# wondras/ld-decode

Hardware: AMD Instinct MI355X
Metric: RF Msamples/s (40 MSPS NTSC, full RF->.tbc decode) (higher is better)
Workload: dtype f64

## Files before the change

include/ldgpu.h:

```cpp
#ifndef LDGPU_H
#define LDGPU_H

#include <stdint.h>
#include <stddef.h>

#ifdef __cplusplus
extern "C" {
#endif

#define LDG_OK 0
#define LDG_EINVAL (-1)
#define LDG_EDEVICE (-2)
#define LDG_ENOMEM (-3)
#define LDG_ESTATE (-4)

#define LDG_SYSTEM_NTSC 0
#define LDG_SYSTEM_PAL 1

#define LDG_FMT_U8 0
#define LDG_FMT_S16 1
#define LDG_FMT_R30 2
#define LDG_FMT_LDS 3

#define LDG_FS_VALID 0
// ... 74 lines not shown
int ldg_stream_release(ldg_ctx* ctx, int64_t below_sample);
int ldg_stream_seek(ldg_ctx* ctx, int64_t first_sample);
int ldg_stream_window(ldg_ctx* ctx, int64_t* out4);
int ldg_stream_stats(ldg_ctx* ctx, double* out, int n);
int ldg_stream_close(ldg_ctx* ctx);

int ldg_decode_reads(ldg_ctx* ctx, int n, const int64_t* read_starts, const double* mtf, const int32_t* slots,
                     ldg_field_info* info);
int ldg_decode_reads_async(ldg_ctx* ctx, int n, const int64_t* read_starts, const double* mtf,
                           const int32_t* slots);
#define LDG_READ_FULL 1
#define LDG_READ_PROBE 2
int ldg_decode_reads_async2(ldg_ctx* ctx, int n, const int64_t* read_starts, const double* mtf,
                            const int32_t* slots, uint8_t* full);
int ldg_set_video_cut(ldg_ctx* ctx, int64_t out_samples);
int ldg_decode_reads_wait(ldg_ctx* ctx, ldg_field_info* info);

int ldg_field_audio(ldg_ctx* ctx, int n, const int32_t* slots, const double* offsets, int16_t* pcm,
                    int64_t pcm_stride, int32_t* counts, double* next_offsets);

int ldg_field_audio_async(ldg_ctx* ctx, int n, const int32_t* slots, const double* offsets);
int ldg_field_audio_collect(ldg_ctx* ctx, int16_t* pcm, int64_t pcm_stride, int32_t* counts, double* next_offsets);

int ldg_archive_fields(ldg_ctx* ctx, int n, const int32_t* slots, int64_t first);
int ldg_archive_audio(ldg_ctx* ctx, int n, const int64_t* entries, const double* offsets, int16_t* pcm,
                      int64_t pcm_stride, int32_t* counts, double* next_offsets);
int ldg_audio_offsets(double o0, int64_t n, const double* linecounts, double line_period, double* out);

int ldg_assemble_frames(ldg_ctx* ctx, int n, const int32_t* top_slots, const int32_t* bottom_slots,
                        uint16_t* out, int out_is_device);
// ... 105 lines not shown
```

ld-decode_amd/csrc/abi.inc:

```
#include <hip/hip_runtime.h>
#include <algorithm>
#include <chrono>
#include <thread>
#include <cmath>
#include <complex>
#include <cstdio>
#include <cstring>
#include <map>
#include <string>
#include <vector>

namespace {

using namespace ldg;

struct DevBuf {
  void* p = nullptr;
  size_t n = 0;
};

}

static inline comb::CombOpt comb_defaults() {
  comb::CombOpt c;
// ... 834 lines not shown
  return check_launch(ctx, "ldg_k_demod");
}

static int launch_chain(ldg_ctx* ctx, hipStream_t st, int n, const int32_t* M_) {
  const SysConst C = ctx->C;
  if (!(ctx->skip >> 0 & 1)) LDG_LAUNCH_ON(st, "sync_walk", ldg_k_sync_walk, n * SEG_K, 64, M_, ctx->d_reads, ctx->video, ctx->vread, ctx->vchan, C,
             ctx->d_status, ctx->d_npos, ctx->d_npk, ctx->d_nlv, ctx->d_ncnt, ctx->d_stile, ctx->d_sst,
             ctx->d_sbits);
  if (!(ctx->skip >> 1 & 1)) LDG_LAUNCH_ON(st, "sync", ldg_k_sync, n, 64, M_, ctx->d_reads, ctx->video, ctx->vread, ctx->vchan, C, ctx->d_recs,
             ctx->d_peaks, ctx->d_status, ctx->d_npos, ctx->d_npk, ctx->d_nlv, ctx->d_ncnt, ctx->d_stile,
             ctx->d_sst, ctx->d_sbits, (ctx->skip >> 9) & 1);
  if (!(ctx->skip >> 2 & 1)) LDG_LAUNCH_ON(st, "linelocs", ldg_k_linelocs, n, 64, M_, ctx->video, ctx->vread, ctx->vchan, C, ctx->d_recs,
             ctx->d_peaks, ctx->d_lines, ctx->d_bad, ctx->d_sst, ctx->d_sbits);
  const dim3 g_lines((unsigned)(C.frame_lines / 2 + 5), (unsigned)n), g_rows((unsigned)(C.frame_lines / 2 + 1), (unsigned)n);
  if (!(ctx->skip >> 3 & 1)) LDG_LAUNCH_ON(st, "hsync_lines", ldg_k_hsync_lines, g_lines, 64, M_, ctx->video, ctx->vread, ctx->vchan, C,
             ctx->d_recs, ctx->d_lines, ctx->d_bad);
  if (!(ctx->skip >> 4 & 1)) LDG_LAUNCH_ON(st, "hsync_field", ldg_k_hsync_field, n, 256, M_, C, ctx->d_recs, ctx->d_lines, ctx->d_bad);
  if (!(ctx->skip >> 5 & 1)) LDG_LAUNCH_ON(st, "philips", ldg_k_philips, n, 192, M_, ctx->video, ctx->vread, ctx->vchan, C, ctx->d_recs,
             ctx->d_lines, ctx->d_reads);
  if (int rc = check_launch(ctx, "field kernels")) return rc;
  if (ctx->system == 0) {
    for (int pass = 0; pass < 2; pass++) {
      if (!(ctx->skip >> 6 & 1)) LDG_LAUNCH_ON(st, "burst_lines", ldg_k_burst_lines, g_lines, 64, M_, ctx->video, ctx->vread, ctx->vchan, C,
                 ctx->d_recs, ctx->d_lines, ctx->d_blevel, pass, ctx->d_bst, ctx->d_reads);
      if (!(ctx->skip >> 7 & 1)) LDG_LAUNCH_ON(st, "burst_field", ldg_k_burst_field, n, 64, M_, ctx->video, ctx->vread, ctx->vchan,
                 ctx->d_recs, ctx->d_lines, ctx->d_blevel, C, pass, ctx->d_bst);
    }
  } else {
    LDG_LAUNCH_ON(st, "pilot_lines", ldg_k_pilot_lines, g_lines, 64, M_, ctx->video, ctx->vread, ctx->vchan, C,
               ctx->d_recs, ctx->d_lines, ctx->d_scratch, ctx->d_reads);
    LDG_LAUNCH_ON(st, "pilot_field", ldg_k_pilot_field, n, 256, M_, ctx->d_recs, ctx->d_lines, C, ctx->d_scratch);
  }
  if (!(ctx->skip >> 8 & 1)) LDG_LAUNCH_ON(st, "final_lines", ldg_k_final_lines, g_rows, FINAL_NT, M_, ctx->video, ctx->vread, ctx->vchan, C,
             ctx->d_recs, ctx->d_lines, ctx->d_blevel, ctx->d_pic, ctx->pic_stride, ctx->d_reads);
  if (int rc = check_launch(ctx, "tbc kernels")) return rc;
  return LDG_OK;
}

struct HostProf {
  bool on = getenv("LDG_HOSTPROF") != nullptr;
  std::chrono::steady_clock::time_point t0 = std::chrono::steady_clock::now(), t = t0;
  char buf[512];
  int len = 0;
  void mark(const char* what) {
    if (!on) return;
    const auto u = std::chrono::steady_clock::now();
// ... 14 lines not shown

int ldg_set_video_cut(ldg_ctx* ctx, int64_t out_samples) {
  if (!ctx || out_samples < 0) return LDG_EINVAL;
  ctx->video_cut = out_samples;
  return LDG_OK;
}

static void read_geometry(ReadDesc& r, int64_t start) {
  r.readsample = start;
  r.end = start + READLEN + 1;
  r.s0 = start > BLOCKCUT ? start - BLOCKCUT : 0;
  r.n_out = (int32_t)(r.end - r.s0 + 1);
  r.n_blocks = (int32_t)((r.end - r.s0 + BLOCKSTEP - 1) / BLOCKSTEP);
  r.n_audio = (int32_t)((r.end - r.s0) / AUDIO_DIV1 + 1);
  r.n_audio2 = r.n_audio / AUDIO_DIV2;
}

static int probe_halfwin(const SysConst& C) { return (int)(3 * (int64_t)C.linelen / 10); }

int ldg_decode_reads_async2(ldg_ctx* ctx, int n, const int64_t* read_starts, const double* mtf,
                            const int32_t* slots, uint8_t* full) {
  if (!ctx || n <= 0 || n > ctx->max_reads || !read_starts || !mtf) return LDG_EINVAL;
  if (ctx->ncalls >= ldg_ctx::MAX_CALLS) {
    ctx->err = "too many decodes outstanding";
    return LDG_ESTATE;
  }
  if (!ctx->have_filters || !ctx->cap) {
    ctx->err = "filters or capture not set";
    return LDG_ESTATE;
  }
// ... 73 lines not shown
      if (!(full[i] & LDG_READ_PROBE)) continue;
      ReadDesc pr = nr[i];
      const int64_t r0 = nr[i].readsample - PROBE_C;
      if (!(ctx->stages & 1) || r0 - BLOCKCUT < ctx->cap_first ||
          r0 - BLOCKCUT + BLOCKLEN > ctx->cap_first + ctx->cap_nsamp) {
        full[i] &= (uint8_t)~LDG_READ_PROBE;
        continue;
      }
      read_geometry(pr, r0);
      pr.end = r0 + BLOCKSTEP + 64;
      pr.n_out = (int32_t)(pr.end - pr.s0 + 1);
      pr.n_blocks = 1;
      pr.n_audio = (int32_t)((pr.end - pr.s0) / AUDIO_DIV1 + 1);
      pr.n_audio2 = pr.n_audio / AUDIO_DIV2;
      pr.vcut = 0;
      hpr[np] = pr;
      hps[np++] = smap[i];
    }
  int32_t* dps = ctx->d_psm + (size_t)ci * R;
  hipStream_t sp = ctx->sprep;
  if (call.demod_recorded) LDG_TRY(hipStreamWaitEvent(sp, call.ev_demod, 0));
  LDG_LAUNCH_ON(sp, "new_reads", ldg_k_new_reads, (n + 255) / 256, 256, hnr, hsm, n, dsm, ctx->d_reads, ctx->d_status);
  if (np) LDG_LAUNCH_ON(sp, "new_reads", ldg_k_new_reads, (np + 255) / 256, 256, hpr, hps, np, dps, ctx->d_preads,
                        ctx->d_status);
    LDG_LAUNCH_ON(sp, "rf_table", ldg_k_rf_table, dim3(BLOCKLEN / 256, (unsigned)tm.size()), 256, ctx->rfvideo, ctx->mtf,
                  ctx->mtf_logabs, ctx->mtf_arg, htm, ctx->rf_cur);
  if (int rc = check_launch(ctx, "ldg_k_rf_table")) return rc;
  LDG_TRY(hipEventRecord(call.ev_prep, sp));
  LDG_TRY(hipStreamWaitEvent(s, call.ev_prep, 0));
  if (ctx->frames_recorded && ctx->frames_demod) LDG_TRY(hipStreamWaitEvent(s, ctx->ev_frames, 0));
// ... 1663 lines not shown
```

ld-decode_amd/csrc/common.hpp:

```cpp
#pragma once
#include <stdint.h>

namespace ldg {

constexpr int BLOCKLEN = 16384;
constexpr int BLOCKCUT = 1024;
constexpr int BLOCKCUT_END = 32;
constexpr int BLOCKSTEP = BLOCKLEN - BLOCKCUT - BLOCKCUT_END;
constexpr int HALF = BLOCKLEN / 2;
constexpr int MAX_BLOCKS_PER_READ = 66;
constexpr int PARK_SLOTS = 2048;
constexpr int PARK_EXTRA = 64;
constexpr int PARK_SCRATCH = PARK_SLOTS + PARK_EXTRA;
constexpr int PARK_TOTAL = PARK_SCRATCH + 1;
constexpr int PARK_OWNERS = PARK_SLOTS + PARK_EXTRA;
constexpr int READLEN = 1000000;
constexpr int MAX_NOUT = READLEN + 1026 + 16;
constexpr int AUDIO_DIV1 = 16;
constexpr int AUDIO_BLOCK = 1024;
constexpr int MAX_NAUDIO = MAX_NOUT / AUDIO_DIV1 + 16;
constexpr int AUDIO_DIV2 = 4;
constexpr int AUDIO2_BLOCK = 4096;
constexpr int MAX_NAUDIO2 = MAX_NAUDIO / AUDIO_DIV2 + 16;
constexpr int MAX_PEAKS = 2048;
// ... 16 lines not shown
  FS_CRASH = 6,
  FS_PENDING = 7,
  FS_MIGRATED = 8,
  FS_VCUT = 9,
};

struct ReadDesc {
  int64_t readsample;
  int64_t s0;
  int64_t end;
  int32_t n_out;
  int32_t n_blocks;
  int32_t n_audio;
  int32_t n_audio2;
  int32_t filt_slot;
  int32_t pad_;
  int64_t vcut;
};

struct SysConst {
  double freq_hz;
  double freq;
  double ire0, hz_ire, vsync_ire;
  double sync_lo, sync_hi;
  double freq_arf;
  double audio_lowfreq;
  double audio_lfreq, audio_rfreq;
  double line_period;
  double fsc_mhz;
  double sy_b0, sy_p;
  double bu_b0, bu_b1, bu_b2, bu_a1, bu_a2;
  int32_t system;
// ... 46 lines not shown
```

ld-decode_amd/csrc/demod.hip:

```cpp
#include <hip/hip_runtime.h>
#include "common.hpp"
#include "fft8k.hpp"
#include "iir.hpp"
#include "chan.hpp"

using namespace ldg;

namespace {

constexpr int T = 1024;
constexpr int M = HALF;

__device__ __forceinline__ double load_sample(const uint8_t* __restrict__ cap, int fmt, int64_t rel) {
  if (fmt == 0) return (double)cap[rel];
  if (fmt == 1) return (double)reinterpret_cast<const int16_t*>(cap)[rel];
  if (fmt == 2) {
    const int64_t w = rel / 3;
    const int sh = 10 * (int)(rel - 3 * w);
    return (double)((reinterpret_cast<const uint32_t*>(cap)[w] >> sh) & 0x3ffu);
  }
  const int64_t g = rel >> 2;
  const int k = (int)(rel & 3);
  const uint8_t* b = cap + 5 * g;
  uint32_t v;
// ... 300 lines not shown
      const int m = tid + T * q;
      X_[m] = make_double2(load_sample(cap, fmt, rel0 + 2 * m), load_sample(cap, fmt, rel0 + 2 * m + 1));
    }
  }
  STAMP(1);
  if (!(kProbe & 8)) fft8k_dif<false>(s_x, tw, twl, tid);
  else __syncthreads();
  STAMP(2);
  const bool park_lost = s_park < 0;
  double2* const park = ospill + (int64_t)(park_lost ? PARK_SCRATCH : s_park) * M;

  {
    Pairs X;
    if (!(kProbe & 64)) split_pairs(X_, twk, tid, X);
    else for (int c = 0; c < 5; c++) { X.a[c] = X_[tid + 1024 * c]; X.b[c] = X.a[c]; }
    {
      const int t = fresh(tid);
      const int a0 = C.audio_lo0;
      const bool mir = t >= 512;
      const int k = mir ? a0 + 1 + (t - 512) : a0 + t;
      const int j = mir ? a0 + 1024 - k : t;
      double2 xk = rsplit(X_[dr_pos(k)], X_[dr_pos(M - k)], tw[k]);
      if (mir) xk = conj2(xk);
      const double2 al = cmul(xk, a_lfilt[j]), ar = cmul(xk, a_rfilt[j]);
      double2* as = aslice + ((int64_t)slot * MAX_BLOCKS_PER_READ + b) * 2048;
      as[j] = al;
      as[1024 + j] = ar;
    }
    __syncthreads();
    const int t = fresh(tid);
#pragma unroll
// ... 81 lines not shown
  const double inv = 1.0 / (double)M;
  double pl1, pt1, p151, p311;
  double2* sx = s_x;
  {
    if (!(kProbe & 32)) merge_pairs(X_, twk, g_05, tid, D);
    STAMP(12);
    double2 zr[8];
    fft8k_dit<true, true>(s_x, tw, twl, tid, zr);
    STAMP(13);
    const int t = fresh(tid);
    pl1 = iir[IIR_P1 + (t & 63)];
    pt1 = iir[IIR_P1 + t];
    p151 = iir[IIR_P1 + scan_d15(t & 63)];
    p311 = iir[IIR_P1 + scan_d31(t & 63)];
    double* o = vout + (int64_t)CH_05 * vchan_stride;
#pragma unroll
    for (int q = 0; q < 8; q++) {
      const int m = t + T * q;
      const double v0 = zr[q].x * inv, v1 = zr[q].y * inv;
      if (!kProbeNoStore) {
        const int p0 = (2 * m - BLOCKCUT_END) & (BLOCKLEN - 1);
        const int pw0 = (2 * (m & ~63) - BLOCKCUT_END) & (BLOCKLEN - 1);
        if (pw0 >= BLOCKCUT && pw0 + 127 < BLOCKCUT + copylen) {
          st_pair(o + p0, make_double2(v0, v1));
        } else {
          const bool in0 = p0 >= BLOCKCUT && p0 < BLOCKCUT + copylen;
          const bool in1 = p0 + 1 >= BLOCKCUT && p0 + 1 < BLOCKCUT + copylen;
          if (in0 && in1) *reinterpret_cast<double2*>(o + p0) = make_double2(v0, v1);
          else if (in0) o[p0] = v0;
          else if (in1) o[p0 + 1] = v1;
        }
      }
      const uint32_t f0 = (v0 >= C.sync_lo && v0 <= C.sync_hi) ? 1u : 0u;
      const uint32_t f1 = (v1 >= C.sync_lo && v1 <= C.sync_hi) ? 1u : 0u;
      int xb = (int)((f0 | (f1 << 1)) << (2 * (t & 7)));
// ... 138 lines not shown
    const double ov = __shfl_xor(best, m);
    const int oi = __shfl_xor(bi, m);
    if (ov > best || (ov == best && oi < bi)) { best = ov; bi = oi; }
  }
  if (lane == 0) {
    if (!eof && best > 0.2) {
      ReadDesc r = reads[slot];
      const int64_t start = preads[slot].readsample + bi;
      r.readsample = start;
      r.end = start + READLEN + 1;
      r.s0 = start > BLOCKCUT ? start - BLOCKCUT : 0;
      r.n_out = (int32_t)(r.end - r.s0 + 1);
      r.n_blocks = (int32_t)((r.end - r.s0 + BLOCKSTEP - 1) / BLOCKSTEP);
      r.n_audio = (int32_t)((r.end - r.s0) / AUDIO_DIV1 + 1);
      r.n_audio2 = r.n_audio / AUDIO_DIV2;
      if (r.n_out <= MAX_NOUT && r.n_blocks <= MAX_BLOCKS_PER_READ) reads[slot] = r;
    }
    status[slot] = 0;
  }
}

constexpr int A1_T = 256;
constexpr int A1_H = A1_T / 2;
constexpr int A1_P = 1024 / A1_H;
extern "C" __global__ __launch_bounds__(A1_T) void ldg_k_audio1(
    const int32_t* __restrict__ smap, const ReadDesc* __restrict__ reads, const double2* __restrict__ tw, SysConst C,
    const double2* __restrict__ aslice, double* __restrict__ audio1, int64_t aread_stride, int64_t achan_stride,
    const int32_t* __restrict__ status) {
  __shared__ double2 s_a[2048];
  const CBuf A_{s_a};
  const int tid = threadIdx.x;
  const int slot = smap[blockIdx.x / MAX_BLOCKS_PER_READ];
  const int b = blockIdx.x % MAX_BLOCKS_PER_READ;
  const ReadDesc rd = reads[slot];
  if (b >= rd.n_blocks || status[slot] == FS_EOF) return;
  const int off = b * BLOCKSTEP;
  const int copylen = (off + (BLOCKLEN - BLOCKCUT) > rd.n_out) ? rd.n_out - off : BLOCKSTEP;
  constexpr double TAU = 6.283185307179586;
  const double2* as = aslice + ((int64_t)slot * MAX_BLOCKS_PER_READ + b) * 2048;
  __shared__ double s_atan[65];
  if (tid < 65) s_atan[tid] = c_atan64[tid];
#pragma unroll
  for (int q = 0; q < 2048 / A1_T; q++) A_[tid + A1_T * q] = as[tid + A1_T * q];
  {
    const int g = tid / A1_H, lt = tid % A1_H;
    const CBuf ga = A_ + (g ? 1024 : 0);
    fft_lds<1024, A1_H, true>(ga, tw, lt);
    double th[A1_P];
#pragma unroll
    for (int e = 0; e < A1_P; e++) {
// ... 13 lines not shown
      const double prev = p ? gth[p - 1] : 0.0;
      const double d = p ? fold_tau(th[e] - prev) : 0.0;
      const double v = d * (C.freq_arf / TAU) + C.audio_lowfreq;
      const int j = p - BLOCKCUT / AUDIO_DIV1;
      if (j >= 0 && j < kept) aout[off / AUDIO_DIV1 + j] = v;
    }
    if (b == rd.n_blocks - 1) {
      const int last = (off + copylen) / AUDIO_DIV1;
      for (int j = last + lt; j < rd.n_audio; j += A1_H) aout[j] = 0.0;
    }
  }
}

constexpr int AUDIO2_JMAX = 4;
constexpr int AUDIO2_WG = 2 * AUDIO2_JMAX;
static_assert((MAX_NAUDIO - 2 * (BLOCKLEN - 64 * AUDIO_DIV2) + (BLOCKLEN - 64 * AUDIO_DIV2) - 1) /
                          (BLOCKLEN - 64 * AUDIO_DIV2) + 2 <= AUDIO2_JMAX,
              "audio phase 2: a read needs more blocks than the grid has");
extern "C" __global__ __launch_bounds__(1024) void ldg_k_audio2(
    const int32_t* __restrict__ smap, const ReadDesc* __restrict__ reads, const double2* __restrict__ tw, const double2* __restrict__ lpf2,
    const double* __restrict__ audio1, int64_t aread_stride, int64_t achan_stride,
    double* __restrict__ audio2, int64_t a2read_stride, int64_t a2chan_stride, const int32_t* __restrict__ status) {
  __shared__ double2 s_x[M];
  __shared__ double2 s_tw[TW_LDS_N];
  const CBuf X_{s_x};
  const int tid = threadIdx.x;
  s_tw[tw_lds_pos(tid)] = tw[2 * tid];
  const TwLds twl{s_tw};
  const int ch = blockIdx.x & 1;
  const int j = (blockIdx.x >> 1) & (AUDIO2_JMAX - 1);
  const int slot = smap[blockIdx.x / AUDIO2_WG];
  if (status[slot] == FS_EOF) return;
  const ReadDesc rd = reads[slot];
  const int n_in = rd.n_audio, n_out = rd.n_audio2;
  constexpr int SKIP = 64;
  constexpr int JUMP = BLOCKLEN - SKIP * AUDIO_DIV2;
  const int span = n_in - JUMP - JUMP;
  const int n_mid = span > 0 ? (span + JUMP - 1) / JUMP : 0;
  if (j > n_mid + 1) return;
  const int start = (j == 0) ? 0 : (j <= n_mid ? JUMP * j : n_in - BLOCKLEN - 1);
  const double* src = audio1 + (int64_t)slot * aread_stride + (int64_t)ch * achan_stride + start;
#pragma unroll
  for (int q = 0; q < 8; q++) {
    const int m = tid + T * q;
    X_[m] = make_double2(src[2 * m], src[2 * m + 1]);
  }
  fft8k_dif<false>(s_x, tw, twl, tid);
  double2 xa, xb, xc = make_double2(0, 0);
  {
    const int k1 = tid, k2 = tid + 1024;
    xa = rsplit(X_[dr_pos(k1)], X_[dr_pos((M - k1) & (M - 1))], tw[k1]);
    xb = rsplit(X_[dr_pos(k2)], X_[dr_pos(M - k2)], tw[k2]);
    if (tid == 0) xc = rsplit(X_[dr_pos(2048)], X_[dr_pos(M - 2048)], tw[2048]);
  }
  __syncthreads();
// ... 2 lines not shown
    const double2 xs[2] = {xa, xb};
#pragma unroll
    for (int e = 0; e < 2; e++) {
      const int k = ks[e];
      X_[k] = cmul(xs[e], lpf2[k]);
      if (k >= 1) {
        const int jj = AUDIO2_BLOCK - k;
        X_[jj] = cmul(conj2(xs[e]), lpf2[jj]);
      }
    }
    if (tid == 0) X_[2048] = cmul(conj2(xc), lpf2[2048]);
  }
  fft_lds<AUDIO2_BLOCK, 512, true>(X_, tw, tid);
  double* dst = audio2 + (int64_t)slot * a2read_stride + (int64_t)ch * a2chan_stride;
  const double scale = 1.0 / (double)AUDIO2_BLOCK / (double)AUDIO_DIV2;
  const int last_start = n_out - (AUDIO2_BLOCK - SKIP);
#pragma unroll
  for (int e = 0; e < 4; e++) {
    const int p = tid + 1024 * e;
    const double v = X_[p].x * scale;
    int o;
    if (j == 0) {
      o = p;
      if (o >= last_start) continue;
    } else if (j <= n_mid) {
      if (p < SKIP) continue;
      o = AUDIO2_BLOCK + (AUDIO2_BLOCK - SKIP) * (j - 1) + (p - SKIP);
      if (o >= last_start) continue;
    } else {
      if (p < SKIP) continue;
      o = last_start + (p - SKIP);
// ... 33 lines not shown
```

ld-decode_amd/csrc/field.hip:

```cpp
#include <hip/hip_runtime.h>
#include "common.hpp"
#include "field_rec.hpp"
#include "pyops.hpp"
#include "chan.hpp"

using namespace ldg;

namespace {

constexpr int SEG_K = 64;
constexpr int SEG_NMAX = 96;

struct SyncView {
  const int32_t* pk;
  const double* lv;
  int np;
  double med, tol;
  __device__ bool regular(int64_t n, int64_t len_ds, bool& err) const {
    if (n >= np) return false;
    int64_t idx;
    if (!py_index(n, np, idx)) { err = true; return false; }
    if (pk[idx] > len_ds) return false;
    return inrange(lv[idx], med - tol, med + tol);
  }
// ... 651 lines not shown
        zc2 += ((double)py_int(zc) - (fr * 1));
        if (fabs(zc2 - zc) < (fr / 4)) v = zc2;
        else lb = true;
      }
    }
  } else {
    lb = true;
  }
  out = v;
  flag = lb ? 1 : 0;
}
}

extern "C" __global__ __launch_bounds__(64) void ldg_k_hsync_lines(
    const int32_t* __restrict__ smap, const double* __restrict__ video, int64_t vread_stride, int64_t vchan_stride,
    SysConst C, FieldRec* __restrict__ recs, double* __restrict__ lines, int8_t* __restrict__ bad) {
  prio_latency();

  __shared__ double s_tmp[20];
  const int lane = threadIdx.x;
  const int slot = smap[blockIdx.y];
  const int i = blockIdx.x;
  FieldRec* R = recs + slot;
  const double* L1 = lines + (int64_t)slot * LINES_STRIDE + LL1 * MAX_LINES;
  double* L2 = lines + (int64_t)slot * LINES_STRIDE + LL2 * MAX_LINES;
  int8_t* B = bad + (int64_t)slot * MAX_LINES;
  const int status = R->status, nl = R->nlines;
  const int64_t len = R->n_out;
  const double v = L1[i];
  const int lbi = B[i];
  asm volatile("" ::"v"(v), "v"(status), "v"(nl), "v"(lbi));
  if (status != FS_PENDING) return;
  if (i >= nl) return;
  const double* d05 = video + (int64_t)slot * vread_stride + (int64_t)CH_05 * vchan_stride;
  const bool lb = lbi != 0;
  double out;
  int flag;
  hsync_line(d05, len, C, i, v, lb, lane, s_tmp, out, flag);
  if (lane == 0) { L2[i] = out; B[i] = (int8_t)flag; }
}

extern "C" __global__ __launch_bounds__(256) void ldg_k_hsync_field(const int32_t* __restrict__ smap, SysConst C,
                                                                   FieldRec* __restrict__ recs,
                                                                   double* __restrict__ lines,
                                                                   int8_t* __restrict__ bad) {
  prio_latency();

  __shared__ double s_v[MAX_LINES];
  __shared__ int8_t s_bad[MAX_LINES];
  __shared__ int s_err;
// ... 133 lines not shown
```

ld-decode_amd/csrc/tbc.hip:

```cpp
#include <hip/hip_runtime.h>
#include "common.hpp"
#include "field_rec.hpp"
#include "pyops.hpp"
#include "chan.hpp"

using namespace ldg;

namespace {

constexpr int SPL_MAXN = 2816;
constexpr int64_t SPL_HARDN = 1 << 24;
constexpr int LINE_GROUPS = (MAX_LINES + 63) / 64;

struct CTab { double v[17]; };
constexpr CTab make_ctab() {
  CTab t{};
  double c = 0.25;
  for (int i = 0; i < 17; i++) { t.v[i] = c; c = 1.0 / (4.0 - c); }
  return t;
}
__constant__ CTab g_ctab = make_ctab();
constexpr double kCtInf = make_ctab().v[16];
constexpr double kSixth = 1.0 / 6.0;
__device__ __forceinline__ double ctab(int64_t t) { return g_ctab.v[t < 16 ? t : 16]; }
// ... 280 lines not shown
  float out_level = lf;
  if (((lv / hzs) > 30) || (sd / hzs) < 3) {
    out_level = 0.0f;
  } else if (!(nF < 3 || nT < 3)) {
    const double mF = pw_sum(s_g[0] + 1, nF - 2) / (double)(nF - 2);
    const double mT = pw_sum(s_g[1] + 1, nT - 2) / (double)(nT - 2);
    if (l % 2) { p0 = 2 - mT; p1 = 2 - mF; }
    else { p0 = 2 - mF; p1 = 2 - mT; }
  }
  lvl[l] = out_level;
  pv0[l] = p0;
  pv1[l] = p1;
  return 0;
}

constexpr float BURST_LINE_LONG = -1.0f;

}

extern "C" __global__ __launch_bounds__(64) void ldg_k_burst_lines(
    const int32_t* __restrict__ smap, const double* __restrict__ video, int64_t vread_stride, int64_t vchan_stride, SysConst C,
    FieldRec* __restrict__ recs, double* __restrict__ lines, float* __restrict__ blevel, int pass,
    const double4* __restrict__ bst, const ReadDesc* __restrict__ reads) {
  prio_latency();

  __shared__ BurstLDS S;
  __shared__ double s_ba[40], s_t[40], s_g[2][40];
  const int lane = threadIdx.x;
  const int slot = smap[blockIdx.y];
  const int l = blockIdx.x;
// ... 18 lines not shown
  }
  const int rc = burst_line<false>(video, vread_stride, vchan_stride, C, R->n_out, bst, slot, l, b0, b1, lane, S, s_ba, s_t,
                                   s_g, lvl, pv0, pv1);
  if (rc < 0 && lane == 0) {
    if (rc == -2) lvl[l] = BURST_LINE_LONG;
    else R->status = FS_TBC;
  }
#ifdef LDG_STAMPS
  if (lane == 0 && rc == 0 && blockIdx.x < KST_BLOCKS) g_kst[4][blockIdx.x][7] = __builtin_readcyclecounter();
#endif
}

extern "C" __global__ __launch_bounds__(64) void ldg_k_burst_field(
    const int32_t* __restrict__ smap, const double* __restrict__ video, int64_t vread_stride, int64_t vchan_stride,
    FieldRec* __restrict__ recs, double* __restrict__ lines, float* __restrict__ blevel, SysConst C, int pass,
    const double4* __restrict__ bst) {
  prio_latency();

  __shared__ double s_c0[512], s_c1[512];
  __shared__ int s_hist[256];
  __shared__ double s_lo[MAX_LINES];
  __shared__ float s_lvl[MAX_LINES];
  __shared__ int s_g;
  const int lane = threadIdx.x;
  const int slot = smap[blockIdx.x];
  FieldRec* R = recs + slot;
  if (R->status != FS_PENDING) return;
  const int nl = R->nlines;
  double* LN = lines + (int64_t)slot * LINES_STRIDE;
  const double* li = LN + (pass == 0 ? LL2 : LL3) * MAX_LINES;
  double* lo = LN + (pass == 0 ? LL3 : LL4) * MAX_LINES;
// ... 67 lines not shown
      uint64_t mm = m;
      while (mm) {
        const int j = l0 + __ffsll((unsigned long long)mm) - 1;
        mm &= mm - 1;
        s_lo[j] = (s_lo[j - 1] + s_lo[j + 1]) / 2;
      }
    }
    __syncthreads();
  }
  const double shift = (90 + 1.5) * (3.141592653589793 / 180);
  const double c = (shift - 8) * K;
  double* lf = LN + LLF * MAX_LINES;
  for (int l = lane; l < nl; l += 64) {
    lo[l] = s_lo[l];
    lvl[l] = s_lvl[l];
    if (pass == 1) lf[l] = (s_lo[l] + 0) + c;
  }
  if (lane == 0) R->burst_group = g;
#ifdef LDG_STAMPS
  if (blockIdx.x < KST_BLOCKS) g_kst[2][blockIdx.x][3] = __builtin_readcyclecounter();
#endif
}

constexpr int FINAL_NT = 256;
constexpr int FINAL_CHMAX = ((SPL_MAXN + FINAL_NT - 1) / FINAL_NT) | 1;
struct FinalLDS {
  double ms[SPL_MAXN + 1];
  double ct[17];
  double ra[FINAL_NT / 16], rb[FINAL_NT / 16];
  double m1, mn1;
};
constexpr int FINAL_WCAP = 1280;
using FinalWinLDS = SplineLDS<FINAL_NT, FINAL_WCAP>;
// ... 452 lines not shown
      }
      __syncthreads();
      const uint64_t r = *key;
      __syncthreads();
      return r;
    }
    __syncthreads();
  }
  return prefix;
}
}

extern "C" __global__ __launch_bounds__(256) void ldg_k_pilot_field(const int32_t* __restrict__ smap,
                                                                    FieldRec* __restrict__ recs,
                                                                    double* __restrict__ lines, SysConst C,
                                                                    double* __restrict__ scratch) {
  prio_latency();

  constexpr int NALL = 8192;
  static_assert(MAX_LINES <= 512, "two lines per thread");
  __shared__ double s_all[NALL];
  __shared__ int s_wsum[4];
  __shared__ int s_hist[256];
  __shared__ int s_sel[3];
  __shared__ uint64_t s_key;
  const int tid = threadIdx.x, lane = tid & 63, w = tid >> 6;
  const int slot = smap[blockIdx.x];
  FieldRec* R = recs + slot;
  if (R->status != FS_PENDING) return;
  const int nl = R->nlines;
  double* P = pilot_base(scratch, slot);
// ... 15 lines not shown
  for (int q = 0; q < c0; q++)
    if (off + q < NALL) s_all[off + q] = P[(int64_t)l0 * PILOT_MAX + q];
  off += c0;
  for (int q = 0; q < c1; q++)
    if (off + q < NALL) s_all[off + q] = P[(int64_t)l1 * PILOT_MAX + q];
  __syncthreads();
  const int n = total < NALL ? total : NALL;
  double med = __builtin_nan("");
  if (n > 0) {
    med = dkey_val(block_kth_key(s_all, n, (n - 1) / 2, tid, s_hist, s_sel, &s_key));
    if (!(n & 1)) med = (med + dkey_val(block_kth_key(s_all, n, n / 2, tid, s_hist, s_sel, &s_key))) / 2.0;
  }
  const double tgt = inrange(med, 0.25, 0.75) ? .5 : 0;
  const double* ll = lines + (int64_t)slot * LINES_STRIDE + LL2 * MAX_LINES;
  double* lf = lines + (int64_t)slot * LINES_STRIDE + LLF * MAX_LINES;
  for (int l = tid; l < nl; l += 256) {
    double v = ll[l];
    if (meta[3 * l + 0] > 0) v += (tgt - meta[3 * l + 2]) * (C.freq / 3.75) * .25;
    lf[l] = v;
  }
}
```

ld-decode_amd/ldgpu/native.py:

```python
import ctypes as C
import os

import numpy as np

HERE = os.path.dirname(os.path.abspath(__file__))
LIB_PATH = os.path.join(HERE, 'libldgpu.so')

LDG_OK = 0
FS_VALID, FS_NO_VSYNC, FS_SHORT, FS_LINELOCS, FS_TBC, FS_EOF, FS_CRASH, FS_PENDING, FS_MIGRATED, FS_VCUT = range(10)
VBI_NONE = -2147483648
READ_FULL, READ_PROBE = 1, 2
LOG_NO_VSYNC = 1 << 16
MAX_VSYNCS = 16

EXPORTS = ['ldg_create', 'ldg_destroy', 'ldg_last_error', 'ldg_set_filters', 'ldg_set_capture',
           'ldg_decode_reads', 'ldg_field_audio', 'ldg_assemble_frames', 'ldg_debug_read',
           'ldg_comb_ntsc', 'ldg_comb_reset', 'ldg_version', 'ldg_device_count', 'ldg_profile_enable',
           'ldg_profile_read', 'ldg_synth_capture', 'ldg_capture_download', 'ldg_comb_ntsc_async', 'ldg_sync', 'ldg_demod_isolated', 'ldg_demod_isolated_ex', 'ldg_comb_set_opts', 'ldg_output_async', 'ldg_output_wait',
           'ldg_host_alloc', 'ldg_host_free',
           'ldg_archive_fields', 'ldg_archive_audio', 'ldg_decode_reads_async', 'ldg_decode_reads_async2',
           'ldg_set_video_cut', 'ldg_decode_reads_wait',
           'ldg_field_audio_async', 'ldg_field_audio_collect', 'ldg_comb_ntsc3d', 'ldg_cx_create', 'ldg_cx_destroy', 'ldg_cx_process', 'ldg_comb_pal', 'ldg_comb_set_state', 'ldg_profile_spans', 'ldg_profile_spans_union', 'ldg_profile_span_table',
           'ldg_audio_offsets', 'ldg_comb_async', 'ldg_debug_rf_table',
           'ldg_stream_open', 'ldg_stream_release', 'ldg_stream_seek', 'ldg_stream_window', 'ldg_stream_stats',
           'ldg_stream_close', 'ldg_device_memory',
           'ldg_dropout_defaults', 'ldg_set_dropout_opts', 'ldg_field_dropouts',
           'ldg_stack_frames', 'ldg_conceal_frames', 'ldg_stack_stats']
STACK_MAX_SOURCES = 16
STACK_MODES = {'median': 0, 'mean': 1, 'smart-mean': 2}
STACK_STATS = ('h2d_s', 'kernel_s', 'd2h_s', 'calls')
FRAME_SHAPE = {'NTSC': (525, 910), 'PAL': (625, 1135)}
MAX_DROPOUTS_PER_LINE = 8
MAX_LINES = 320
STREAM_STATS = ('bytes_read', 'read_s', 'chunks', 'launch_waits', 'launch_wait_s', 'space_wait_s', 'seeks',
                'ring_bytes', 'chunk_bytes', 'stage_wait_s')

# ... 105 lines not shown
    lib.ldg_debug_read.restype = C.c_int64
    lib.ldg_debug_rf_table.argtypes = [vp, C.c_double, vp]
    lib.ldg_comb_ntsc.argtypes = [vp, C.c_int, vp, vp, C.c_int]
    lib.ldg_comb_reset.argtypes = [vp]
    lib.ldg_comb_set_opts.argtypes = [vp, C.POINTER(CombOpts)]
    lib.ldg_output_async.argtypes = [vp, C.c_int, vp, vp, vp, vp]
    lib.ldg_output_wait.argtypes = [vp]
    lib.ldg_host_alloc.argtypes = [C.c_int64, C.POINTER(vp)]
    lib.ldg_host_free.argtypes = [vp]
    lib.ldg_comb_ntsc_async.argtypes = [vp, C.c_int]
    lib.ldg_comb_async.argtypes = [vp, C.c_int]
    lib.ldg_comb_ntsc3d.argtypes = [vp, C.c_int, vp, vp, C.POINTER(C.c_int), C.c_double, C.c_double]
    lib.ldg_decode_reads_async.argtypes = [vp, C.c_int, vp, vp, vp]
    lib.ldg_decode_reads_async2.argtypes = [vp, C.c_int, vp, vp, vp, vp]
    lib.ldg_set_video_cut.argtypes = [vp, C.c_int64]
    lib.ldg_decode_reads_wait.argtypes = [vp, vp]
    lib.ldg_archive_fields.argtypes = [vp, C.c_int, vp, C.c_int64]
    lib.ldg_archive_audio.argtypes = [vp, C.c_int, vp, vp, vp, C.c_int64, vp, vp]
    lib.ldg_sync.argtypes = [vp]
    lib.ldg_demod_isolated.argtypes = [vp, C.c_int, vp, C.c_int, C.POINTER(C.c_double)]
    lib.ldg_demod_isolated_ex.argtypes = [vp, C.c_int, vp, C.c_int, C.c_int, C.POINTER(C.c_double)]
    lib.ldg_profile_enable.argtypes = [vp, C.c_int]
    lib.ldg_profile_read.argtypes = [vp, C.POINTER(KernelStat), C.c_int]
    lib.ldg_profile_spans.argtypes = [vp, C.POINTER(C.c_double), C.POINTER(C.c_int64)]
    lib.ldg_profile_spans_union.argtypes = [vp, C.POINTER(C.c_double), C.POINTER(C.c_int64)]
    lib.ldg_profile_span_table.argtypes = [vp, vp, C.c_int]
    lib.ldg_synth_capture.argtypes = [vp, C.POINTER(SynthParams), C.POINTER(C.c_double), C.POINTER(C.c_double),
                                      C.POINTER(C.c_uint32), C.c_int64]
    lib.ldg_capture_download.argtypes = [vp, vp, C.c_int64, C.c_int64]
    lib.ldg_capture_download.restype = C.c_int64
# ... 472 lines not shown
                                               nframes), 'ldg_synth_capture')

    def capture_copy_to_device(self, dst_ptr, offset, nbytes):
        n = self.lib.ldg_capture_download(self.h, C.c_void_p(dst_ptr), offset, nbytes)
        if n != nbytes:
            raise LDGError('ldg_capture_download -> %d' % n)

    def capture_download(self, offset, nbytes):
        a = np.zeros(nbytes, dtype=np.uint8)
        n = self.lib.ldg_capture_download(self.h, a.ctypes.data_as(C.c_void_p), offset, nbytes)
        if n < 0:
            raise LDGError('ldg_capture_download -> %d' % n)
        return a[:n]


def audio_offsets(o0, linecounts, line_period):
    lc = np.ascontiguousarray(linecounts, dtype=np.float64)
    out = np.zeros(lc.size + 1, dtype=np.float64)
    rc = load().ldg_audio_offsets(float(o0), lc.size, lc.ctypes.data, float(line_period), out.ctypes.data)
    if rc != 0:
        raise IndexError('downscale_audio: empty tick range (the reference raises here)')
    return out.tolist()


class CXExpander:

    def __init__(self):
        self.lib = load()
        h = C.c_void_p()
        if self.lib.ldg_cx_create(C.byref(h)) != LDG_OK:
# ... 15 lines not shown
```

Before: 23530.

## Skip demod audio and 0.5 MHz video tail blocks past the video cut

Adds a tail plan computed per read from the video cut, which marks the last audio-phase-2 block and the audio-phase-1 blocks beyond a cut point as dead so their kernels return early. It also skips storing the 0.5 MHz video channel past the cut. Fields whose hsync or audio line spans reach past the cut are now flagged FS_VCUT so the skipped tail is never consumed. This trades extra per-field checks and synchronisation in the field kernels for less FFT and audio work on read tails, and it risks changing which fields get migrated or re-read.

```diff
diff --git a/include/ldgpu.h b/include/ldgpu.h
--- a/include/ldgpu.h
+++ b/include/ldgpu.h
@@ -112,6 +112,9 @@
 int ldg_decode_reads_async2(ldg_ctx* ctx, int n, const int64_t* read_starts, const double* mtf,
                             const int32_t* slots, uint8_t* full);
 int ldg_set_video_cut(ldg_ctx* ctx, int64_t out_samples);
+
+int ldg_tail_plan(int64_t n_out, int64_t n_audio, int64_t n_audio2, int64_t vcut, int64_t out[5]);
+int ldg_audio_reach(const double* lines, int nlines, int linecount, double linelen, double out[2]);
 int ldg_decode_reads_wait(ldg_ctx* ctx, ldg_field_info* info);
 
 int ldg_field_audio(ldg_ctx* ctx, int n, const int32_t* slots, const double* offsets, int16_t* pcm,
diff --git a/ld-decode_amd/csrc/abi.inc b/ld-decode_amd/csrc/abi.inc
--- a/ld-decode_amd/csrc/abi.inc
+++ b/ld-decode_amd/csrc/abi.inc
@@ -872,7 +872,7 @@
              ctx->d_peaks, ctx->d_lines, ctx->d_bad, ctx->d_sst, ctx->d_sbits);
   const dim3 g_lines((unsigned)(C.frame_lines / 2 + 5), (unsigned)n), g_rows((unsigned)(C.frame_lines / 2 + 1), (unsigned)n);
   if (!(ctx->skip >> 3 & 1)) LDG_LAUNCH_ON(st, "hsync_lines", ldg_k_hsync_lines, g_lines, 64, M_, ctx->video, ctx->vread, ctx->vchan, C,
-             ctx->d_recs, ctx->d_lines, ctx->d_bad);
+             ctx->d_recs, ctx->d_lines, ctx->d_bad, ctx->d_reads);
   if (!(ctx->skip >> 4 & 1)) LDG_LAUNCH_ON(st, "hsync_field", ldg_k_hsync_field, n, 256, M_, C, ctx->d_recs, ctx->d_lines, ctx->d_bad);
   if (!(ctx->skip >> 5 & 1)) LDG_LAUNCH_ON(st, "philips", ldg_k_philips, n, 192, M_, ctx->video, ctx->vread, ctx->vchan, C, ctx->d_recs,
              ctx->d_lines, ctx->d_reads);
@@ -882,12 +882,13 @@
       if (!(ctx->skip >> 6 & 1)) LDG_LAUNCH_ON(st, "burst_lines", ldg_k_burst_lines, g_lines, 64, M_, ctx->video, ctx->vread, ctx->vchan, C,
                  ctx->d_recs, ctx->d_lines, ctx->d_blevel, pass, ctx->d_bst, ctx->d_reads);
       if (!(ctx->skip >> 7 & 1)) LDG_LAUNCH_ON(st, "burst_field", ldg_k_burst_field, n, 64, M_, ctx->video, ctx->vread, ctx->vchan,
-                 ctx->d_recs, ctx->d_lines, ctx->d_blevel, C, pass, ctx->d_bst);
+                 ctx->d_recs, ctx->d_lines, ctx->d_blevel, C, pass, ctx->d_bst, ctx->d_reads);
     }
   } else {
     LDG_LAUNCH_ON(st, "pilot_lines", ldg_k_pilot_lines, g_lines, 64, M_, ctx->video, ctx->vread, ctx->vchan, C,
                ctx->d_recs, ctx->d_lines, ctx->d_scratch, ctx->d_reads);
-    LDG_LAUNCH_ON(st, "pilot_field", ldg_k_pilot_field, n, 256, M_, ctx->d_recs, ctx->d_lines, C, ctx->d_scratch);
+    LDG_LAUNCH_ON(st, "pilot_field", ldg_k_pilot_field, n, 256, M_, ctx->d_recs, ctx->d_lines, C, ctx->d_scratch,
+               ctx->d_reads);
   }
   if (!(ctx->skip >> 8 & 1)) LDG_LAUNCH_ON(st, "final_lines", ldg_k_final_lines, g_rows, FINAL_NT, M_, ctx->video, ctx->vread, ctx->vchan, C,
              ctx->d_recs, ctx->d_lines, ctx->d_blevel, ctx->d_pic, ctx->pic_stride, ctx->d_reads);
@@ -932,6 +933,41 @@
   r.n_blocks = (int32_t)((r.end - r.s0 + BLOCKSTEP - 1) / BLOCKSTEP);
   r.n_audio = (int32_t)((r.end - r.s0) / AUDIO_DIV1 + 1);
   r.n_audio2 = r.n_audio / AUDIO_DIV2;
+  const TailPlan tp = tail_plan(r.n_audio, r.n_audio2, r.vcut);
+  r.acut1 = tp.acut1;
+  r.acut2 = tp.acut2;
+}
+
+int ldg_tail_plan(int64_t n_out, int64_t n_audio, int64_t n_audio2, int64_t vcut, int64_t out[5]) {
+  if (!out || n_out < 0 || n_out > MAX_NOUT || n_audio < 0 || n_audio > MAX_NAUDIO || n_audio2 < 0 ||
+      n_audio2 > MAX_NAUDIO2 || vcut < 0)
+    return LDG_EINVAL;
+  const TailPlan tp = tail_plan((int)n_audio, (int)n_audio2, vcut > 0 ? vcut : INT64_MAX);
+  const int n_blocks = (int)((n_out - 1 + BLOCKSTEP - 1) / BLOCKSTEP), n_mid = a2_n_mid((int)n_audio);
+  out[0] = tp.acut1 == ACUT_NONE ? -1 : tp.acut1;
+  out[1] = tp.acut2 == ACUT_NONE ? -1 : tp.acut2;
+  out[2] = out[3] = out[4] = 0;
+  for (int j = 0; j <= n_mid + 1; j++) out[2] += !a2_block_dead(j, n_mid, tp.acut2);
+  for (int b = 0; b < n_blocks; b++) {
+    out[3] += !a1_block_dead(b, tp.acut1);
+    out[4] += !(vcut > 0 && (int64_t)b * BLOCKSTEP >= vcut);
+  }
+  return LDG_OK;
+}
+
+int ldg_audio_reach(const double* lines, int nlines, int linecount, double linelen, double out[2]) {
+  if (!lines || !out || nlines <= 0 || nlines > MAX_LINES || linecount < 0) return LDG_EINVAL;
+  double lo = __builtin_inf(), hi = -__builtin_inf();
+  for (int il = 0; il <= audio_last_line(nlines, linecount); il++) {
+    double a, b;
+    audio_line_span(lines, nlines, il, linelen, a, b);
+    if (!(a == a)) { lo = hi = a; break; }
+    lo = std::min(lo, a);
+    hi = std::max(hi, b);
+  }
+  out[0] = lo;
+  out[1] = hi;
+  return LDG_OK;
 }
 
 static int probe_halfwin(const SysConst& C) { return (int)(3 * (int64_t)C.linelen / 10); }
@@ -1035,6 +1071,7 @@
       pr.n_audio = (int32_t)((pr.end - pr.s0) / AUDIO_DIV1 + 1);
       pr.n_audio2 = pr.n_audio / AUDIO_DIV2;
       pr.vcut = 0;
+      pr.acut1 = pr.acut2 = ACUT_NONE;
       hpr[np] = pr;
       hps[np++] = smap[i];
     }
diff --git a/ld-decode_amd/csrc/common.hpp b/ld-decode_amd/csrc/common.hpp
--- a/ld-decode_amd/csrc/common.hpp
+++ b/ld-decode_amd/csrc/common.hpp
@@ -54,8 +54,10 @@
   int32_t n_audio;
   int32_t n_audio2;
   int32_t filt_slot;
+  int32_t acut1;
+  int64_t vcut;
+  int32_t acut2;
   int32_t pad_;
-  int64_t vcut;
 };
 
 struct SysConst {
diff --git a/ld-decode_amd/csrc/demod.hip b/ld-decode_amd/csrc/demod.hip
--- a/ld-decode_amd/csrc/demod.hip
+++ b/ld-decode_amd/csrc/demod.hip
@@ -3,6 +3,7 @@
 #include "fft8k.hpp"
 #include "iir.hpp"
 #include "chan.hpp"
+#include "tail.hpp"
 
 using namespace ldg;
 
@@ -338,7 +339,7 @@
     Pairs X;
     if (!(kProbe & 64)) split_pairs(X_, twk, tid, X);
     else for (int c = 0; c < 5; c++) { X.a[c] = X_[tid + 1024 * c]; X.b[c] = X.a[c]; }
-    {
+    if (!(CUT && a1_block_dead(b, rd.acut1))) {
       const int t = fresh(tid);
       const int a0 = C.audio_lo0;
       const bool mir = t >= 512;
@@ -450,11 +451,12 @@
     p151 = iir[IIR_P1 + scan_d15(t & 63)];
     p311 = iir[IIR_P1 + scan_d31(t & 63)];
     double* o = vout + (int64_t)CH_05 * vchan_stride;
+    const bool st05 = !kProbeNoStore && !(CUT && (int64_t)off >= rd.vcut);
 #pragma unroll
     for (int q = 0; q < 8; q++) {
       const int m = t + T * q;
       const double v0 = zr[q].x * inv, v1 = zr[q].y * inv;
-      if (!kProbeNoStore) {
+      if (st05) {
         const int p0 = (2 * m - BLOCKCUT_END) & (BLOCKLEN - 1);
         const int pw0 = (2 * (m & ~63) - BLOCKCUT_END) & (BLOCKLEN - 1);
         if (pw0 >= BLOCKCUT && pw0 + 127 < BLOCKCUT + copylen) {
@@ -623,6 +625,9 @@
       r.n_blocks = (int32_t)((r.end - r.s0 + BLOCKSTEP - 1) / BLOCKSTEP);
       r.n_audio = (int32_t)((r.end - r.s0) / AUDIO_DIV1 + 1);
       r.n_audio2 = r.n_audio / AUDIO_DIV2;
+      const TailPlan tp = tail_plan(r.n_audio, r.n_audio2, r.vcut);
+      r.acut1 = tp.acut1;
+      r.acut2 = tp.acut2;
       if (r.n_out <= MAX_NOUT && r.n_blocks <= MAX_BLOCKS_PER_READ) reads[slot] = r;
     }
     status[slot] = 0;
@@ -643,6 +648,7 @@
   const int b = blockIdx.x % MAX_BLOCKS_PER_READ;
   const ReadDesc rd = reads[slot];
   if (b >= rd.n_blocks || status[slot] == FS_EOF) return;
+  if (a1_block_dead(b, rd.acut1)) return;
   const int off = b * BLOCKSTEP;
   const int copylen = (off + (BLOCKLEN - BLOCKCUT) > rd.n_out) ? rd.n_out - off : BLOCKSTEP;
   constexpr double TAU = 6.283185307179586;
@@ -686,8 +692,7 @@
 
 constexpr int AUDIO2_JMAX = 4;
 constexpr int AUDIO2_WG = 2 * AUDIO2_JMAX;
-static_assert((MAX_NAUDIO - 2 * (BLOCKLEN - 64 * AUDIO_DIV2) + (BLOCKLEN - 64 * AUDIO_DIV2) - 1) /
-                          (BLOCKLEN - 64 * AUDIO_DIV2) + 2 <= AUDIO2_JMAX,
+static_assert((MAX_NAUDIO - 2 * A2_JUMP + A2_JUMP - 1) / A2_JUMP + 2 <= AUDIO2_JMAX,
               "audio phase 2: a read needs more blocks than the grid has");
 extern "C" __global__ __launch_bounds__(1024) void ldg_k_audio2(
     const int32_t* __restrict__ smap, const ReadDesc* __restrict__ reads, const double2* __restrict__ tw, const double2* __restrict__ lpf2,
@@ -705,12 +710,11 @@
   if (status[slot] == FS_EOF) return;
   const ReadDesc rd = reads[slot];
   const int n_in = rd.n_audio, n_out = rd.n_audio2;
-  constexpr int SKIP = 64;
-  constexpr int JUMP = BLOCKLEN - SKIP * AUDIO_DIV2;
-  const int span = n_in - JUMP - JUMP;
-  const int n_mid = span > 0 ? (span + JUMP - 1) / JUMP : 0;
+  constexpr int SKIP = A2_SKIP;
+  const int n_mid = a2_n_mid(n_in);
   if (j > n_mid + 1) return;
-  const int start = (j == 0) ? 0 : (j <= n_mid ? JUMP * j : n_in - BLOCKLEN - 1);
+  if (a2_block_dead(j, n_mid, rd.acut2)) return;
+  const int start = a2_block_start(j, n_mid, n_in);
   const double* src = audio1 + (int64_t)slot * aread_stride + (int64_t)ch * achan_stride + start;
 #pragma unroll
   for (int q = 0; q < 8; q++) {
@@ -743,7 +747,7 @@
   fft_lds<AUDIO2_BLOCK, 512, true>(X_, tw, tid);
   double* dst = audio2 + (int64_t)slot * a2read_stride + (int64_t)ch * a2chan_stride;
   const double scale = 1.0 / (double)AUDIO2_BLOCK / (double)AUDIO_DIV2;
-  const int last_start = n_out - (AUDIO2_BLOCK - SKIP);
+  const int last_start = a2_last_start(n_out);
 #pragma unroll
   for (int e = 0; e < 4; e++) {
     const int p = tid + 1024 * e;
diff --git a/ld-decode_amd/csrc/field.hip b/ld-decode_amd/csrc/field.hip
--- a/ld-decode_amd/csrc/field.hip
+++ b/ld-decode_amd/csrc/field.hip
@@ -689,7 +689,8 @@
 
 extern "C" __global__ __launch_bounds__(64) void ldg_k_hsync_lines(
     const int32_t* __restrict__ smap, const double* __restrict__ video, int64_t vread_stride, int64_t vchan_stride,
-    SysConst C, FieldRec* __restrict__ recs, double* __restrict__ lines, int8_t* __restrict__ bad) {
+    SysConst C, FieldRec* __restrict__ recs, double* __restrict__ lines, int8_t* __restrict__ bad,
+    const ReadDesc* __restrict__ reads) {
   prio_latency();
 
   __shared__ double s_tmp[20];
@@ -709,6 +710,14 @@
   if (i >= nl) return;
   const double* d05 = video + (int64_t)slot * vread_stride + (int64_t)CH_05 * vchan_stride;
   const bool lb = lbi != 0;
+  {
+    const int64_t vcut = reads[slot].vcut;
+    const double s = i < 9 ? v - 200 : v, fr = C.freq;
+    if (vcut != INT64_MAX && !(s - 2 * fr - 2 >= 0 && s + 400 + 3 * fr + 2 < (double)vcut)) {
+      if (lane == 0) R->status = FS_VCUT;
+      return;
+    }
+  }
   double out;
   int flag;
   hsync_line(d05, len, C, i, v, lb, lane, s_tmp, out, flag);
diff --git a/ld-decode_amd/csrc/tail.hpp b/ld-decode_amd/csrc/tail.hpp
--- /dev/null
+++ b/ld-decode_amd/csrc/tail.hpp
@@ -0,0 +1,62 @@
+#pragma once
+#include <stdint.h>
+
+#include "common.hpp"
+
+#if defined(__HIPCC__) || defined(__CUDACC__)
+#define LDG_HD __host__ __device__
+#else
+#define LDG_HD
+#endif
+
+namespace ldg {
+
+constexpr int32_t ACUT_NONE = INT32_MAX;
+constexpr int A2_SKIP = 64;
+constexpr int A2_JUMP = BLOCKLEN - A2_SKIP * AUDIO_DIV2;
+constexpr int A2_KEEP = AUDIO2_BLOCK - A2_SKIP;
+constexpr int A1_STEP = BLOCKSTEP / AUDIO_DIV1;
+static_assert(BLOCKSTEP % AUDIO_DIV1 == 0, "a demod block keeps whole audio-1 samples");
+
+LDG_HD inline int a2_n_mid(int n_in) {
+  const int span = n_in - A2_JUMP - A2_JUMP;
+  return span > 0 ? (span + A2_JUMP - 1) / A2_JUMP : 0;
+}
+LDG_HD inline int a2_block_start(int j, int n_mid, int n_in) {
+  return j == 0 ? 0 : (j <= n_mid ? A2_JUMP * j : n_in - BLOCKLEN - 1);
+}
+LDG_HD inline int a2_last_start(int n_out2) { return n_out2 - A2_KEEP; }
+
+struct TailPlan {
+  int32_t acut1;
+  int32_t acut2;
+};
+
+LDG_HD inline TailPlan tail_plan(int n_audio, int n_audio2, int64_t vcut) {
+  TailPlan p{ACUT_NONE, ACUT_NONE};
+  if (vcut <= 0 || vcut == INT64_MAX) return p;
+  const int last_start = a2_last_start(n_audio2);
+  if (last_start <= 0 || n_audio - BLOCKLEN - 1 < 0) return p;
+  const int64_t vcut2 = (vcut + AUDIO_DIV1 * AUDIO_DIV2 - 1) / (AUDIO_DIV1 * AUDIO_DIV2);
+  if (vcut2 > last_start) return p;
+  p.acut2 = last_start;
+  p.acut1 = a2_n_mid(n_audio) * A2_JUMP + BLOCKLEN;
+  return p;
+}
+
+LDG_HD inline bool a1_block_dead(int b, int32_t acut1) { return (int64_t)b * A1_STEP >= acut1; }
+LDG_HD inline bool a2_block_dead(int j, int n_mid, int32_t acut2) { return acut2 != ACUT_NONE && j == n_mid + 1; }
+
+LDG_HD inline void audio_line_span(const double* lf, int nl, int il, double linelen, double& lo, double& hi) {
+  const double cur = lf[il];
+  const double nxt = (il + 1 < nl) ? lf[il + 1] : cur + linelen;
+  lo = cur < nxt ? cur : nxt;
+  hi = cur < nxt ? nxt : cur;
+  if (!(cur == cur) || !(nxt == nxt)) lo = hi = cur + nxt;
+}
+LDG_HD inline int audio_last_line(int nl, int linecount) { return linecount + 1 < nl - 1 ? linecount + 1 : nl - 1; }
+LDG_HD inline bool audio_span_ok(double lo, double hi, int32_t acut2) {
+  return lo >= 0.0 && hi < (double)(AUDIO_DIV1 * AUDIO_DIV2) * (double)acut2;
+}
+
+}
diff --git a/ld-decode_amd/csrc/tbc.hip b/ld-decode_amd/csrc/tbc.hip
--- a/ld-decode_amd/csrc/tbc.hip
+++ b/ld-decode_amd/csrc/tbc.hip
@@ -1,6 +1,7 @@
 #include <hip/hip_runtime.h>
 #include "common.hpp"
 #include "field_rec.hpp"
+#include "tail.hpp"
 #include "pyops.hpp"
 #include "chan.hpp"
 
@@ -318,6 +319,20 @@
   return 0;
 }
 
+__device__ __forceinline__ bool audio_reach_bad(const double* s_lf, int nl, int lc, const SysConst& C, int32_t acut2,
+                                                int tid, int nt) {
+  bool bad = false;
+  if (acut2 != ACUT_NONE) {
+    const int last = audio_last_line(nl, lc);
+    for (int il = tid; il <= last; il += nt) {
+      double a, b;
+      audio_line_span(s_lf, nl, il, (double)C.linelen, a, b);
+      bad |= !audio_span_ok(a, b, acut2);
+    }
+  }
+  return bad;
+}
+
 constexpr float BURST_LINE_LONG = -1.0f;
 
 }
@@ -366,7 +381,7 @@
 extern "C" __global__ __launch_bounds__(64) void ldg_k_burst_field(
     const int32_t* __restrict__ smap, const double* __restrict__ video, int64_t vread_stride, int64_t vchan_stride,
     FieldRec* __restrict__ recs, double* __restrict__ lines, float* __restrict__ blevel, SysConst C, int pass,
-    const double4* __restrict__ bst) {
+    const double4* __restrict__ bst, const ReadDesc* __restrict__ reads) {
   prio_latency();
 
   __shared__ double s_c0[512], s_c1[512];
@@ -464,9 +479,18 @@
   for (int l = lane; l < nl; l += 64) {
     lo[l] = s_lo[l];
     lvl[l] = s_lvl[l];
-    if (pass == 1) lf[l] = (s_lo[l] + 0) + c;
+    if (pass == 1) {
+      const double f = (s_lo[l] + 0) + c;
+      lf[l] = f;
+      s_lo[l] = f;
+    }
   }
   if (lane == 0) R->burst_group = g;
+  if (pass == 1) {
+    __syncthreads();
+    if (__syncthreads_or(audio_reach_bad(s_lo, nl, R->linecount, C, reads[slot].acut2, lane, 64)) && lane == 0)
+      R->status = FS_VCUT;
+  }
 #ifdef LDG_STAMPS
   if (blockIdx.x < KST_BLOCKS) g_kst[2][blockIdx.x][3] = __builtin_readcyclecounter();
 #endif
@@ -949,7 +973,8 @@
 extern "C" __global__ __launch_bounds__(256) void ldg_k_pilot_field(const int32_t* __restrict__ smap,
                                                                     FieldRec* __restrict__ recs,
                                                                     double* __restrict__ lines, SysConst C,
-                                                                    double* __restrict__ scratch) {
+                                                                    double* __restrict__ scratch,
+                                                                    const ReadDesc* __restrict__ reads) {
   prio_latency();
 
   constexpr int NALL = 8192;
@@ -995,9 +1020,14 @@
   const double tgt = inrange(med, 0.25, 0.75) ? .5 : 0;
   const double* ll = lines + (int64_t)slot * LINES_STRIDE + LL2 * MAX_LINES;
   double* lf = lines + (int64_t)slot * LINES_STRIDE + LLF * MAX_LINES;
+  __syncthreads();
   for (int l = tid; l < nl; l += 256) {
     double v = ll[l];
     if (meta[3 * l + 0] > 0) v += (tgt - meta[3 * l + 2]) * (C.freq / 3.75) * .25;
     lf[l] = v;
-  }
-}
+    s_all[l] = v;
+  }
+  __syncthreads();
+  if (__syncthreads_or(audio_reach_bad(s_all, nl, R->linecount, C, reads[slot].acut2, tid, 256)) && tid == 0)
+    R->status = FS_VCUT;
+}
diff --git a/ld-decode_amd/ldgpu/native.py b/ld-decode_amd/ldgpu/native.py
--- a/ld-decode_amd/ldgpu/native.py
+++ b/ld-decode_amd/ldgpu/native.py
@@ -19,7 +19,7 @@
            'ldg_profile_read', 'ldg_synth_capture', 'ldg_capture_download', 'ldg_comb_ntsc_async', 'ldg_sync', 'ldg_demod_isolated', 'ldg_demod_isolated_ex', 'ldg_comb_set_opts', 'ldg_output_async', 'ldg_output_wait',
            'ldg_host_alloc', 'ldg_host_free',
            'ldg_archive_fields', 'ldg_archive_audio', 'ldg_decode_reads_async', 'ldg_decode_reads_async2',
-           'ldg_set_video_cut', 'ldg_decode_reads_wait',
+           'ldg_set_video_cut', 'ldg_tail_plan', 'ldg_audio_reach', 'ldg_decode_reads_wait',
            'ldg_field_audio_async', 'ldg_field_audio_collect', 'ldg_comb_ntsc3d', 'ldg_cx_create', 'ldg_cx_destroy', 'ldg_cx_process', 'ldg_comb_pal', 'ldg_comb_set_state', 'ldg_profile_spans', 'ldg_profile_spans_union', 'ldg_profile_span_table',
            'ldg_audio_offsets', 'ldg_comb_async', 'ldg_debug_rf_table',
            'ldg_stream_open', 'ldg_stream_release', 'ldg_stream_seek', 'ldg_stream_window', 'ldg_stream_stats',
@@ -155,6 +155,8 @@
     lib.ldg_decode_reads_async.argtypes = [vp, C.c_int, vp, vp, vp]
     lib.ldg_decode_reads_async2.argtypes = [vp, C.c_int, vp, vp, vp, vp]
     lib.ldg_set_video_cut.argtypes = [vp, C.c_int64]
+    lib.ldg_tail_plan.argtypes = [C.c_int64, C.c_int64, C.c_int64, C.c_int64, vp]
+    lib.ldg_audio_reach.argtypes = [vp, C.c_int, C.c_int, C.c_double, vp]
     lib.ldg_decode_reads_wait.argtypes = [vp, vp]
     lib.ldg_archive_fields.argtypes = [vp, C.c_int, vp, C.c_int64]
     lib.ldg_archive_audio.argtypes = [vp, C.c_int, vp, vp, vp, C.c_int64, vp, vp]
@@ -657,6 +659,24 @@
         return a[:n]
 
 
+def tail_plan(n_out, n_audio, n_audio2, vcut):
+    out = np.zeros(5, dtype=np.int64)
+    rc = load().ldg_tail_plan(int(n_out), int(n_audio), int(n_audio2), int(vcut), out.ctypes.data)
+    if rc != 0:
+        raise ValueError('ldg_tail_plan: %d' % rc)
+    a1, a2, l2, l1, l05 = (int(v) for v in out)
+    return (None if a1 < 0 else a1, None if a2 < 0 else a2, l2, l1, l05)
+
+
+def audio_reach(lines, linecount, linelen):
+    ll = np.ascontiguousarray(lines, dtype=np.float64)
+    out = np.zeros(2, dtype=np.float64)
+    rc = load().ldg_audio_reach(ll.ctypes.data, ll.size, int(linecount), float(linelen), out.ctypes.data)
+    if rc != 0:
+        raise ValueError('ldg_audio_reach: %d' % rc)
+    return float(out[0]), float(out[1])
+
+
 def audio_offsets(o0, linecounts, line_period):
     lc = np.ascontiguousarray(linecounts, dtype=np.float64)
     out = np.zeros(lc.size + 1, dtype=np.float64)
```

After: 23790, median of 6. 1.01x the previous value.
